# erthward/geonomics

Measured on AMD Instinct MI355X. Metric: individual-timesteps/sec, higher is better.
Workload: dtype u64

## Files before the change

### geonomics_amd/csrc/gnx_api.hip

```cpp
#include <cmath>
#include <cstdarg>
#include <algorithm>
#include <atomic>
#include <chrono>
#include "gnx_internal.h"
#include "gnx_rng.h"
#include "gnx_compact.h"

static thread_local char g_err[1024] = "";

void gnx_set_error(const char* fmt, ...) {
  va_list ap;
  va_start(ap, fmt);
  vsnprintf(g_err, sizeof(g_err), fmt, ap);
  va_end(ap);
}

extern "C" const char* gnx_last_error(void) { return g_err; }

extern "C" int gnx_words_per_hom(int32_t L) {
  int w = (L + 63) / 64;
  return ((w + 15) / 16) * 16;
}

// ... 980 lines not shown
  for (int t = 0; t < h->cfg.n_traits; ++t)
    if (h->traits[t].n_loci == 0) {
      gnx_set_error("trait %d not set (gnx_set_trait)", t);
      return 1;
    }
  return 0;
}

extern "C" int gnx_pop_dynamics_mate(gnx_state* h, int32_t burn) {
  GNXCHK(need_params(h));
  GNXCHK(check_recomb_ready(h, burn != 0));
  int64_t P = 0, B = 0;
  h->tile2_mode = false;
  GNXCHK(gnx_l_sort_by_cell(h, true));
  int rc_pairs = gnx_l_find_pairs(h, nullptr, &P, true);
  GNXCHK(gnx_wait_permute_rest(h));
  GNXCHK(rc_pairs);
  if (P > 0 && !h->spl_P.valid)
    GNXCHK(gnx_l_density(h, P, h->mid_x, h->mid_y, &h->spl_P, nullptr));
  GNXCHK(gnx_l_mate(h, burn != 0, false, 0, &B));
  h->last_births = B;
  return 0;
}

extern "C" int gnx_pop_dynamics_die(gnx_state* h, int32_t burn, int32_t with_selection) {
  GNXCHK(need_params(h));
  int64_t D = 0;
  GNXCHK(gnx_l_density_N(h));
  GNXCHK(gnx_l_death_probs(h, with_selection != 0 && !burn));
  GNXCHK(gnx_l_mortality(h, nullptr, &D));
  h->last_deaths = D;
  return 0;
}

extern "C" int gnx_pop_dynamics(gnx_state* h, int32_t burn, int32_t with_selection) {
  GNXCHK(gnx_pop_dynamics_mate(h, burn));
  return gnx_pop_dynamics_die(h, burn, with_selection);
}

struct GnxStepTimer {
  std::chrono::steady_clock::time_point t0 = std::chrono::steady_clock::now();
  bool count;
  explicit GnxStepTimer(bool c) : count(c) {}
  ~GnxStepTimer() {
    if (gnx_host_times()) {
      g_host_step_s += std::chrono::duration<double>(std::chrono::steady_clock::now() - t0).count();
      if (count) ++g_host_steps;
    }
  }
};

extern "C" int gnx_step_begin(gnx_state* h, int32_t burn) {
  GNXCHK(need_params(h));
  GNXCHK(check_recomb_ready(h, burn != 0));
  GnxStepTimer timer(true);
  if (h->mort_wait || h->pairs_wait) {
    gnx_set_error("gnx_step_begin: the previous step of this handle was not finished (gnx_step_end)");
    return 1;
  }
  h->tot[0] += 1;
  h->tot[1] += h->N - h->n_ghost;
  h->last_xo_births = 0;
  h->step_burn = burn != 0;
  h->tile2_mode = false;
  if (h->moved_ahead) {
    GNXCHK(gnx_move_ahead_join(h));
  } else if (h->sp.move) {
    h->move_writes_keys = h->sp.mating_radius >= 0;
    int rc = gnx_l_move(h, true, nullptr, nullptr, nullptr, nullptr, true);
    h->move_writes_keys = false;
    GNXCHK(rc);
  } else {
    GNXCHK(gnx_l_age(h));
  }
  GNXCHK(gnx_l_sort_by_cell(h, true));
  int rc_pairs = gnx_l_find_pairs_enqueue(h, nullptr, true);
  GNXCHK(gnx_wait_permute_rest(h));
  return rc_pairs;
}

extern "C" int gnx_step_mid(gnx_state* h, int32_t burn, int32_t with_selection) {
  GnxStepTimer timer(false);
  int64_t P = 0, B = 0;
  GNXCHK(gnx_l_find_pairs_finish(h, &P));
  if (P > 0 && !h->spl_P.valid)
    GNXCHK(gnx_l_density(h, P, h->mid_x, h->mid_y, &h->spl_P, nullptr));
  GNXCHK(gnx_l_mate(h, burn != 0, false, 0, &B));
  h->last_births = B;
  GNXCHK(gnx_l_density_N(h));
  GNXCHK(gnx_l_death_probs(h, with_selection != 0 && !burn));
  return gnx_l_mortality_enqueue(h, nullptr);
}

extern "C" int gnx_step_end(gnx_state* h, int32_t burn) {
  GnxStepTimer timer(false);
  int64_t D = 0;
  GNXCHK(gnx_l_mortality_finish(h, &D));
  h->last_deaths = D;
  h->step += 1;
  h->tot[2] += h->last_births;
  h->tot[3] += h->last_deaths;
  if (!burn) h->tot[4] += h->last_xo_births;
  return 0;
}

extern "C" int gnx_step(gnx_state* h, int32_t burn, int32_t with_selection) {
  GNXCHK(gnx_step_begin(h, burn));
  GNXCHK(gnx_step_mid(h, burn, with_selection));
  return gnx_step_end(h, burn);
}

extern "C" int gnx_step_many(gnx_state** hs, int32_t n, int32_t burn, int32_t with_selection) {
  for (int k = 0; k < n; ++k) GNXCHK(gnx_step_begin(hs[k], burn));
  for (int k = 0; k < n; ++k) GNXCHK(gnx_step_mid(hs[k], burn, with_selection));
  for (int k = 0; k < n; ++k) GNXCHK(gnx_step_end(hs[k], burn));
  return 0;
}

extern "C" int gnx_set_id_order(gnx_state* h, int32_t mode) {
  if (mode != 0 && mode != 1) {
    gnx_set_error("gnx_set_id_order: 0 (hash cell, focal id) or 1 (virtual-tile-major)");
    return 1;
  }
  if (mode == 1 && (h->cfg.W % 8 || h->cfg.H % 8)) {
    gnx_set_error("tile-major offspring ids need landscape dimensions divisible by 8");
    return 1;
  }
  if (mode == 1) GNXCHK(gnx_vt_buffers(h));
  h->id_order = mode;
  h->cfg_epoch += 1;
  return 0;
}

extern "C" int gnx_totals(gnx_state* h, int64_t* out) {
  for (int k = 0; k < 6; ++k) out[k] = h->tot[k];
  return 0;
}

extern "C" int gnx_reset_totals(gnx_state* h) {
  for (int k = 0; k < 6; ++k) h->tot[k] = 0;
  return 0;
}

extern "C" int gnx_path_counts(gnx_state* h, int64_t* out, int32_t n) {
  for (int k = 0; k < n; ++k) out[k] = k < GNX_PC_COUNT ? h->pc[k] : 0;
  return GNX_PC_COUNT;
}

extern "C" int gnx_reset_path_counts(gnx_state* h) {
  for (int k = 0; k < GNX_PC_COUNT; ++k) h->pc[k] = 0;
  return 0;
}

__global__ void k_gather_births(int64_t B, int64_t first, GnxSoA s, const int32_t* off_parent,
                                int64_t* child_id, int64_t* parent_id, float* xy) {
  int64_t k = (int64_t)blockIdx.x * blockDim.x + threadIdx.x;
  if (k >= B) return;
  child_id[k] = s.id[first + k];
  parent_id[2 * k] = s.id[off_parent[2 * k]];
  parent_id[2 * k + 1] = s.id[off_parent[2 * k + 1]];
  xy[2 * k] = s.x[first + k];
  xy[2 * k + 1] = s.y[first + k];
}

extern "C" int gnx_last_births(gnx_state* h, int64_t* child_id, int64_t* parent_id, int32_t* keys,
                               uint8_t* starts, float* xy) {
  const int64_t B = h->last_births;
  if (B <= 0) return 0;
  if (B > h->N) {
    gnx_set_error("gnx_last_births: call it between gnx_pop_dynamics_mate and _die");
// ... 457 lines not shown
```

### geonomics_amd/csrc/gnx_internal.h

```cpp
#pragma once
#include <cstring>
#include <cstdint>
#include <cstdio>
#include <cstdlib>
#include <string>
#include <vector>
#include <utility>
#include <hip/hip_runtime.h>
#include "../../include/gnx_hip.h"
#include "gnx_half.h"

#define GNX_MAX_TRAITS 16
#define GNX_MAX_LAYERS 16
#define GNX_DISP_ATTEMPTS 8
#define GNX_SPARSE_MAX_BP 24

void gnx_set_error(const char* fmt, ...);

static inline int gnx_env_int(const char* name, int dflt) {
  const char* v = getenv(name);
  return v ? atoi(v) : dflt;
}
static inline int64_t gnx_dd_max_cap() {
  static const int64_t v = getenv("GNX_DD_MAX_CAP") ? atoll(getenv("GNX_DD_MAX_CAP")) : 600000;
// ... 382 lines not shown
  int32_t* req_count = nullptr;
  bool tiled = false;
  int tile_R = 1, tile_C = 1, tile_r = 0, tile_c = 0;
  gnx_ind_rec* st_rec = nullptr;
  float* st_z = nullptr;
  uint64_t* st_geno = nullptr;
  int64_t* st_slots = nullptr;
  int64_t st_n = 0, st_cap = 0, st_geno_cap = 0;
  bool st_has_geno = false;
  int64_t birth_first_slot = 0;
  int64_t n_req = 0;
  gnx_ind_rec* gp_rec = nullptr;
  float* gp_z = nullptr;
  int64_t* gp_slots = nullptr;
  int64_t gp_cap = 0;
  void* rq_sorted = nullptr;
  int32_t* rq_k = nullptr;
  int64_t rq_cap = 0;
  uint64_t* gam_out = nullptr;
  int32_t* gam_slot = nullptr;
  int64_t gam_cap = 0;
  int64_t* chk = nullptr;
  int64_t tile_evict = 0;
  float evict_box[4]{};
  int64_t n_req_known = -1;
  gnx_ind_rec* gh_rec = nullptr;
  int64_t gh_cap = 0;
  int32_t* route_cnt = nullptr;
  int64_t route_n_mig = 0, route_n_gh = 0;
  int64_t prev_deaths = 0;
  int32_t* h_route_pin = nullptr;
  int32_t* h_route_pin_dev = nullptr;
  std::vector<int64_t> req_by_rank;
  bool tile_req_on_device = false;
  bool tile2_mode = false;
  bool req_cnt_zeroed = false;
  bool tile_pairs_nowait = false;
  bool tile_births_settled = false;

  int32_t* mate = nullptr;
  int32_t* flag = nullptr;
  int32_t* flag2 = nullptr;
  int32_t* scan = nullptr;
  int32_t* pairs = nullptr;
  int32_t* nbirths = nullptr;
  int32_t* boff = nullptr;
  int32_t* off_pair = nullptr;
  int32_t* off_parent = nullptr;
  int32_t* off_keys = nullptr;
  uint8_t* off_start = nullptr;
  uint8_t* keep_in = nullptr;
  float* inj_a = nullptr;
  float* inj_b = nullptr;
  float* mid_x = nullptr;
  float* mid_y = nullptr;
  int64_t n_pairs = 0;
  bool pairs_wait = false;
  int64_t pairs_seq = 0;
  bool pairs_with_top = false, pairs_with_density = false;
  bool mort_wait = false;
  bool mort_xo = false, mort_fill = false, mort_ord_keep = false;
  int mort_has_rows = 0;
  int64_t mort_N = 0;

  GnxLattice lat;
  GnxSpline spl_N, spl_P;
  int32_t* bin_partials = nullptr;
  int32_t* bins_P = nullptr;
  bool bins_zeroed[2]{};
  bool nmax_zeroed = false;
  bool req_zeroed = false;
  int32_t* fb[3]{};
  bool fb_zero[3]{};
  int fb_cur = 0;
  bool fb_adults = false;
  int64_t fb_count = 0;
  unsigned long long* nmax2 = nullptr;
  const unsigned long long* nmax_cur = nullptr;
  bool nmax_ready = false;
  bool last_N_fused = false;
  hipEvent_t ev_pairs = nullptr, ev_latP = nullptr, ev_perm = nullptr, ev_binsN = nullptr;
  bool binsN_inflight = false;
  bool latP_inflight = false;
  bool ord_mode = true;
  bool ord_valid = false;
  int64_t ord_n = 0;
  int ord_cur = 0;
  int32_t* ord[2]{};
  int32_t* newslot = nullptr;
  bool compact_fill = true;
  bool jobs_self_scan = false;
  bool ord_covers_xo = false;
  bool permute_split = true;
  bool perm_rest_inflight = false;
  bool perm_rest_pending = false;
  GnxSoA perm_rest_a{}, perm_rest_b{};
  int64_t perm_rest_N = 0;
  hipEvent_t ev_perm_rest = nullptr;
  bool fb_pending = false;
  const float *fbp_x = nullptr, *fbp_y = nullptr;
  int64_t fbp_N = 0;
  hipEvent_t ev_alive = nullptr;
  int32_t* fill_cnt = nullptr;
  hipEvent_t ev_fill = nullptr;
  int64_t fill_guess = 0;
  uint32_t* cell32 = nullptr;
  uint32_t* keyk[2]{};
  int32_t* valk[2]{};
  void* os_scratch = nullptr;
  uint32_t* os_ktmp = nullptr;
  int32_t* os_vtmp = nullptr;
  int32_t* ord_cnt = nullptr;
  int32_t* ord_off = nullptr;
  hipEvent_t ev_ord = nullptr;
  bool ord_inflight = false;
  bool keys_ordmode = false;
  bool keys_fresh = false;
  bool hist_fresh = false;
  bool holes = false;
  int64_t holes_N = 0;
  RouteGeo* route_geo_dev = nullptr;
  uint64_t route_geo_epoch = 0;
  bool move_counts_routes = false;
  bool move_counted_routes = false;
  bool tile_lazy_ok = false;
  int64_t holes_flagged = 0;
  bool eager_move = false;
  bool move_ahead_ok = false;
  bool moved_ahead = false;
  hipEvent_t ev_moved = nullptr;
  bool e_stale = false;
  bool move_writes_keys = false;
  int n_bin_blocks = 0;
  double* nodes = nullptr;
  double* K_over = nullptr;
  unsigned long long* nmax_bits = nullptr;
  double* p_death = nullptr;
  double* d_cell = nullptr;
  uint8_t* dead_in = nullptr;
  int32_t* counts_rast[2]{};
  int counts_cur = 0;
  bool counts_init = false;
  double* red = nullptr;

  int32_t* blk_cnt = nullptr;
  int32_t* blk_off = nullptr;
  int blk_stride = 0;
  int32_t* cnt_dev = nullptr;
  unsigned int* tickets = nullptr;

  int64_t* h_pin = nullptr;
  int64_t* h_pin_dev = nullptr;
  int64_t pin_seq = 0;
  void* h_stage = nullptr;
  size_t h_stage_bytes = 0;

  void* tile_comm = nullptr;
  GnxDD* dd = nullptr;
  GnxDDRec* dd_ring = nullptr;
  GnxDDRec* dd_ring_dev = nullptr;
  bool dd_active = false;
  int64_t dd_seq = 0;
  int64_t dd_seen = 0;
  int64_t dd_half_est = 0;
  int64_t dd_b_hi = 0;
  int64_t dd_use_hi = 0;
  int64_t dd_gc_seq = 0;
  int64_t dd_top_last = 0, dd_top_seq = 0;
  int64_t dd_est_seq = 0;
  int64_t dd_post_gc = 0;
  bool dd_gc_wait = false;
  void* dd_graph[1]{};
  int32_t dd_err = 0;
  std::vector<int64_t> dd_hist;
  bool dd_hist_closed = false;
  uint64_t cfg_epoch = 1;

  bool profiling = false;
  int profile_only = -1;
  GnxKernelTimer timers[GNX_K_COUNT];
  hipEvent_t ev_open = nullptr;
  std::vector<hipEvent_t> ev_free;
  std::vector<std::pair<hipEvent_t, hipEvent_t>> ev_pending[GNX_K_COUNT];
};

GnxTraitTab gnx_trait_tab(const gnx_state* h);

static inline GnxHalves gnx_halves(const gnx_state* h) {
  return GnxHalves{h->hmap, h->half_free, h->half_top, h->NB, h->BW > 0 ? h->BW : h->W64 / h->NB};
}
int gnx_half_reserve(gnx_state* h, int64_t blocks);
int gnx_gc(gnx_state* h);
static inline const int32_t* gnx_alias_bp(const gnx_state* h) {
  return (h->alias_xo && h->sparse_paths) ? h->bp_off : nullptr;
}
static inline const int32_t* gnx_alias_loci(const gnx_state* h) {
  return (h->alias_xo && h->sparse_paths) ? h->bp_loci : nullptr;
}

int gnx_publish(gnx_state* h, int slot, const int32_t* a, const int32_t* b = nullptr,
                const int32_t* c = nullptr, const int32_t* d = nullptr);

void gnx_time_begin(gnx_state* h, int kernel = -1);
void gnx_time_end(gnx_state* h, int kernel, double bytes);

int gnx_h2d(gnx_state* h, void* dst, const void* src, size_t bytes);
int gnx_d2h(gnx_state* h, void* dst, const void* src, size_t bytes);

int gnx_l_init_population(gnx_state* h, int64_t N);
int gnx_l_gather_e(gnx_state* h, int64_t first, int64_t n);
int gnx_l_age(gnx_state* h);
int gnx_l_move(gnx_state* h, bool inc_age, const float* inj_theta, const float* inj_dist,
               float* out_theta, float* out_dist, bool apply);
int gnx_l_move_ahead(gnx_state* h, int64_t N);
int gnx_move_ahead_join(gnx_state* h);
int gnx_l_sort_by_cell(gnx_state* h, bool split_rest = false);
int gnx_wait_permute_rest(gnx_state* h);
int gnx_permute_rest_launch(gnx_state* h);
int gnx_l_find_pairs(gnx_state* h, const uint8_t* d_keep, int64_t* n_pairs_out,
                     bool with_density = false);
int gnx_l_find_pairs_enqueue(gnx_state* h, const uint8_t* d_keep, bool with_density);
int gnx_l_find_pairs_finish(gnx_state* h, int64_t* n_pairs_out);
int gnx_l_births(gnx_state* h, int64_t* births_out);
int gnx_l_pair_cls(gnx_state* h, int64_t P, bool local);
int gnx_vt_buffers(gnx_state* h);
int gnx_l_mate(gnx_state* h, bool burn, bool inject, int64_t B_inject, int64_t* births_out,
               int64_t id_base = -1, bool tiled = false);
int gnx_l_dispersal_inject(gnx_state* h, int64_t B, int A, const float* d_mx, const float* d_my,
                           const float* d_theta, const float* d_dist, float* d_ox, float* d_oy,
                           int32_t* d_used);
int gnx_l_crossover_all(gnx_state* h, int64_t first_slot, int64_t B);
int gnx_l_crossover_requests(gnx_state* h, int64_t first_slot, int64_t n_req);
int gnx_l_crossover_pending(gnx_state* h, int64_t first_slot, int64_t B);
int gnx_l_crossover_survivors(gnx_state* h, int64_t first_slot, int64_t B, const int32_t* d_alive,
                              const int32_t* d_scan);
int gnx_xo_join(gnx_state* h);
int gnx_xo_flush_deferred(gnx_state* h);
int gnx_xo_launch_pending(gnx_state* h, int site = GNX_PC_XO_FLUSH);
int gnx_xo_wait_inflight(gnx_state* h);
int gnx_xo_prepare_jobs(gnx_state* h, int32_t** zero);
int gnx_xo_wait_wide(gnx_state* h);
double gnx_xo_bytes_per_birth(const gnx_state* h);
int gnx_l_rebuild_sel(gnx_state* h);
int gnx_l_path_sel(gnx_state* h);
int gnx_l_tb_from_rows(gnx_state* h, int64_t first, int64_t n, const int32_t* d_list,
                       const int64_t* d_slots, bool join = true);
int gnx_l_newborn_tb(gnx_state* h, int64_t first_slot, int64_t B);
int gnx_l_phenotype(gnx_state* h, int64_t first_slot, int64_t n, const int32_t* d_list = nullptr);
int gnx_l_assign_genomes(gnx_state* h, const int32_t* d_n_per_site);
int gnx_l_mutate(gnx_state* h, int n, const int64_t* d_slot, const int32_t* d_locus,
                 const uint8_t* d_hom);
int gnx_l_density(gnx_state* h, int64_t n, const float* d_x, const float* d_y, GnxSpline* spl,
                  const double* d_nodes_override, const int32_t* n_dev = nullptr);
struct GnxSetWords {
  int32_t* dst = nullptr;
  int32_t v[4] = {0, 0, 0, 0};
};
struct GnxPubWords {
  int n1 = 0;
  const int32_t* src1 = nullptr;
  int32_t* host1 = nullptr;
  int n2 = 0;
  const int32_t* src2 = nullptr;
  int32_t* host2 = nullptr;
};
int gnx_l_bins(gnx_state* h, int64_t n, const float* d_x, const float* d_y, const uint8_t* d_ghost,
               int32_t* d_bins, const int32_t* n_dev = nullptr, const GnxSetWords* sw = nullptr);
int gnx_l_spline(gnx_state* h, const int32_t* d_bins, GnxSpline* spl,
                 const double* d_nodes_override);
int gnx_l_spline_z(gnx_state* h, const int32_t* d_bins, GnxSpline* spl,
                   const double* d_nodes_override, bool housekeeping);
int gnx_l_raster(gnx_state* h, int which, double* d_out);
int gnx_l_density_N(gnx_state* h);
int gnx_l_lattice_P_async(gnx_state* h, int64_t n_max);
int gnx_bins_adults_launch(gnx_state* h);
void gnx_bins_adults_drop(gnx_state* h);
int gnx_l_bins_adults_async(gnx_state* h, const float* d_x, const float* d_y, int64_t N);
int gnx_wait_latP(gnx_state* h);
bool gnx_fused_bins(const gnx_state* h);
int gnx_l_death_probs(gnx_state* h, bool with_selection);
int gnx_l_mortality(gnx_state* h, const uint8_t* d_dead_inject, int64_t* deaths_out);
int gnx_l_mortality_enqueue(gnx_state* h, const uint8_t* d_dead_inject);
int gnx_l_mortality_finish(gnx_state* h, int64_t* deaths_out);
int gnx_l_spatial_diff(gnx_state* h, double* mean, double* sd, double* sums = nullptr);
int gnx_l_gather_genomes(gnx_state* h, int64_t n, const int64_t* d_slots, uint64_t* d_out);
int gnx_l_scatter_genomes(gnx_state* h, int64_t n, const uint64_t* d_in, int64_t first_slot);

int gnx_dd_l_sort(gnx_state* h, int32_t* d_bins, hipStream_t st);
int gnx_dd_l_pairs(gnx_state* h, int32_t* d_bins, hipStream_t st);
int gnx_dd_l_offspring(gnx_state* h, bool genomes, int32_t* d_bins, hipStream_t st);
int gnx_dd_l_density_N(gnx_state* h, int par, hipStream_t st);
int gnx_dd_l_death_probs(gnx_state* h, bool with_selection, int par, hipStream_t st);
int gnx_dd_l_alive(gnx_state* h, bool xo, int buf, hipStream_t st);
int gnx_dd_l_jobs(gnx_state* h, int buf, hipStream_t st);
int gnx_dd_l_crossover(gnx_state* h, int buf, hipStream_t st);
int gnx_dd_l_fill_lists(gnx_state* h, int has_rows, hipStream_t st);
int gnx_dd_l_fill(gnx_state* h, int has_rows, bool xo, hipStream_t st);
int gnx_dd_l_ord_end(gnx_state* h, int has_rows, bool xo, hipStream_t st);
bool gnx_dd_eligible(const gnx_state* h, bool burn);
int gnx_dd_leave(gnx_state* h);
void gnx_dd_destroy(gnx_state* h);

int gnx_block_scan(gnx_state* h, int K, int64_t n_items, const int32_t* cnt, int32_t* off,
                   int32_t* out, int64_t* host, int64_t seq = 0, hipStream_t st = nullptr,
                   const int32_t* extra = nullptr);
int gnx_os_hist_discard(gnx_state* h, hipStream_t st = nullptr);
bool gnx_l_lattices_tiled(gnx_state* h, bool have_pairs, const GnxPubWords& pub);
void gnx_host_mark(int id);
extern double g_host_step_s, g_host_wait_s;
bool gnx_host_times();
size_t gnx_os_scratch_bytes(size_t n, int end_bit);
size_t gnx_os_words_used64(size_t n, int end_bit);
int gnx_os_sort64_clean(void* scratch, void* tmp, const uint64_t* kin, uint64_t* kout,
                        const int32_t* vin, int32_t* vout, size_t n, int end_bit, hipStream_t s);
size_t gnx_os_words_used(size_t n, int end_bit);
int gnx_os_keys_hist(void* scratch, unsigned int* ticket, int64_t N, int64_t ord_n,
                     const int32_t* ord, const uint32_t* cell32, uint32_t* key, int32_t* val,
                     int end_bit, hipStream_t s, const GnxDD* dd = nullptr, int geometry = 0);
void gnx_os_digits(int end_bit, int* places, int* rb);
int gnx_os_sort32_gather(void* scratch, uint32_t* ktmp, int32_t* vtmp, uint32_t* kout, int32_t* vout,
                         size_t n, int end_bit, const int32_t* ord, int64_t ord_n,
// ... 93 lines not shown
```

### geonomics_amd/csrc/gnx_kernels_genome.hip

```cpp
#include "gnx_internal.h"
#include "gnx_rng.h"
#include "gnx_xo.h"
#include "gnx_half.h"
#include "gnx_tb.h"
#include "gnx_compact.h"

__global__ void __launch_bounds__(256)
k_xo_jobs_all(int64_t B, int64_t first, int32_t* __restrict__ grow,
              const int32_t* __restrict__ off_parent, const int32_t* __restrict__ off_keys,
              const uint8_t* __restrict__ off_start, const int32_t* __restrict__ free_rows,
              int64_t n_free, GnxHalves H, const int32_t* __restrict__ bp_off,
              const int32_t* __restrict__ bp_loci, GnxXoJob* __restrict__ jobs,
              int32_t* __restrict__ n_jobs) {
  const int64_t k = (int64_t)blockIdx.x * blockDim.x + threadIdx.x;
  const bool act = k < B;
  int32_t row = -1;
  if (act) {
    row = free_rows[n_free - 1 - k];
    grow[first + k] = row;
  }
#pragma unroll
  for (int p = 0; p < 2; ++p) {
    const int32_t prow = act ? grow[off_parent[2 * k + p]] : -1;
    gnx_xo_gamete(H, act, row, p, prow, act ? off_keys[2 * k + p] : 0,
// ... 166 lines not shown
        jrec.ph0 = GNX_BLK(pe0[b]);
        jrec.ph1 = GNX_BLK(pe1[b]);
        jrec.dst = dst;
        jrec.ks = (key * 2 + st) | (b << 24);
        jobs[job++] = jrec;
      }
    } else {
      const int hsel = (sel >> b) & 1u;
      const int32_t e = hsel ? pe1[b] : pe0[b];
      H.hmap[lb] = GNX_BLK(e);
      if (e < 0) H.hmap[((int64_t)prow * 2 + hsel) * NB + b] = GNX_BLK(e);
    }
  }
  for (int b = 0; b < NB; ++b)
    H.hmap[((int64_t)row * 2 + 1) * NB + b] = (int32_t)((uint32_t)H.stack[pop - nf0 - b] | GNX_OWN);
}

int gnx_l_crossover_requests(gnx_state* h, int64_t first_slot, int64_t n_req) {
  if (n_req == 0) return 0;
  GNXCHK(gnx_xo_launch_pending(h));
  GNXCHK(xo_wait_buf(h, h->stream, 0));
  GNXCHK(xo_wait_buf(h, h->stream, 1));
  const int buf = h->jobs_cur;
  GNXCHK(gnx_half_reserve(h, 2 * (int64_t)h->NB * n_req));
  HIPCHK(hipMemsetAsync(h->n_jobs_dev[buf], 0, sizeof(int32_t), h->stream));
  h->jobs_inline[buf] = false;
  hipLaunchKernelGGL(k_xo_jobs_req, dim3(gnx_grid(n_req, 256)), dim3(256), 0, h->stream, (int)n_req,
                     first_slot, h->soa[h->cur].grow, h->req_k, h->off_parent, h->off_keys,
                     h->off_start, h->free_rows, h->n_free, gnx_halves(h), gnx_alias_bp(h),
                     gnx_alias_loci(h), (GnxXoJob*)h->jobs[buf], h->n_jobs_dev[buf]);
  if (h->stream2) {
    HIPCHK(hipEventRecord(h->ev_jobs, h->stream));
    HIPCHK(hipStreamWaitEvent(h->stream2, h->ev_jobs, 0));
  }
  gnx_time_begin(h, GNX_K_CROSSOVER);
  GNXCHK(xo_launch(h, h->stream, buf, n_req, false));
  gnx_time_end(h, GNX_K_CROSSOVER, 0.0);
  h->n_free -= n_req;
  return 0;
}

__global__ void k_pending_flags(int64_t N, int64_t first, const int32_t* grow, int32_t* alive,
                                int32_t* cnt3) {
  __shared__ int lds[16];
  const int64_t base = (int64_t)blockIdx.x * GNX_CB;
  bool fx[4];
#pragma unroll
  for (int r = 0; r < 4; ++r) {
    const int64_t i = base + r * 256 + threadIdx.x;
    fx[r] = i < N && i >= first && grow[i] < 0;
    if (i < N) alive[i] = fx[r] ? 2 : 0;
  }
  int rank[4], tot;
  gnx_block_ranks(fx, rank, tot, lds);
  if (threadIdx.x == 0) cnt3[blockIdx.x] = tot;
}

int gnx_l_crossover_pending(gnx_state* h, int64_t first_slot, int64_t B) {
  if (B == 0) return 0;
  GNXCHK(gnx_xo_launch_pending(h));
  GNXCHK(xo_wait_buf(h, h->stream, 0));
  GNXCHK(xo_wait_buf(h, h->stream, 1));
  const int64_t N = h->N;
  const int nb = (int)((N + GNX_CB - 1) / GNX_CB);
  const int buf = h->jobs_cur;
  int32_t* cnt3 = h->blk_cnt + 2 * h->blk_stride;
  int32_t* off3 = h->blk_off + 2 * h->blk_stride;
  hipLaunchKernelGGL(k_pending_flags, dim3(nb), dim3(256), 0, h->stream, N, first_slot,
                     h->soa[h->cur].grow, h->flag, cnt3);
  GNXCHK(gnx_block_scan(h, 1, N, cnt3, off3, h->cnt_dev + 2, h->h_pin_dev + 8));
  GNXCHK(gnx_half_reserve(h, 2 * (int64_t)h->NB * B));
  HIPCHK(hipMemsetAsync(h->n_jobs_dev[buf], 0, sizeof(int32_t), h->stream));
  gnx_launch_xo_jobs_surv(h, first_slot, h->flag, h->blk_off, buf);
  gnx_time_begin(h, GNX_K_CROSSOVER);
  GNXCHK(xo_launch(h, h->stream, buf, 2 * B, false));
  HIPCHK(hipStreamSynchronize(h->stream));
  const int64_t S = h->h_pin[8];
  gnx_time_end(h, GNX_K_CROSSOVER, 0.0);
  h->n_free -= S;
  h->last_xo_births = S;
  return 0;
}

int gnx_xo_launch_pending(gnx_state* h, int site) {
  const int buf = h->xo_ready_buf;
  if (buf < 0) return 0;
  h->xo_ready_buf = -1;
  if (site == GNX_PC_XO_P2 || site == GNX_PC_XO_FLUSH) ++h->pc[site];
  HIPCHK(hipEventRecord(h->ev_jobs, h->stream));
  HIPCHK(hipStreamWaitEvent(h->stream2, h->ev_jobs, 0));
  hipStream_t main = h->stream;
  h->stream = h->stream2;
  const int split = (h->xo_sort_waits && h->xo_split > 0 && h->xo_split < 1024) ? h->xo_split : 0;
  h->xo_last_split = split;
  gnx_time_begin(h, GNX_K_CROSSOVER);
  int rc = xo_launch(h, h->stream2, buf, h->xo_ready_jobs, !h->xo_sort_waits, 0,
                     split ? split : 1024);
  gnx_time_end(h, GNX_K_CROSSOVER, 0.0);
  if (split && !rc) {
    HIPCHK(hipEventRecord(h->ev_xo_wide[buf], h->stream2));
    h->xo_wide_inflight[buf] = true;
    gnx_time_begin(h, GNX_K_CROSSOVER);
    rc = xo_launch(h, h->stream2, buf, h->xo_ready_jobs, true, split, 1024);
    gnx_time_end(h, GNX_K_CROSSOVER_TAIL, 0.0);
  }
  h->stream = main;
  GNXCHK(rc);
  HIPCHK(hipEventRecord(h->ev_xo_done[buf], h->stream2));
  h->xo_inflight[buf] = true;
  h->xo_running = true;
  return 0;
}

int gnx_xo_wait_inflight(gnx_state* h) {
  GNXCHK(xo_wait_buf(h, h->stream, 0));
  GNXCHK(xo_wait_buf(h, h->stream, 1));
  return 0;
}

int gnx_xo_wait_wide(gnx_state* h) {
  for (int buf = 0; buf < 2; ++buf) {
    if (h->xo_wide_inflight[buf]) {
      HIPCHK(hipStreamWaitEvent(h->stream, h->ev_xo_wide[buf], 0));
      h->xo_wide_inflight[buf] = false;
    } else if (!h->xo_last_split) {
      GNXCHK(xo_wait_buf(h, h->stream, buf));
    }
  }
  return 0;
}

int gnx_xo_prepare_jobs(gnx_state* h, int32_t** zero) {
  GNXCHK(gnx_xo_launch_pending(h));
  const int buf = h->jobs_cur;
  GNXCHK(xo_wait_buf(h, h->stream, buf));
  *zero = h->n_jobs_dev[buf];
  return 0;
}

int gnx_l_crossover_survivors(gnx_state* h, int64_t first_slot, int64_t B, const int32_t* d_alive,
                              const int32_t* d_scan) {
  if (B == 0) return 0;
  const int buf = h->jobs_cur;
  gnx_launch_xo_jobs_surv(h, first_slot, d_alive, d_scan, buf);
  HIPCHK(hipGetLastError());
  h->xo_ready_buf = buf;
  h->xo_ready_jobs = 2 * B;
  h->jobs_cur ^= 1;
  if (!h->xo_launch_late || h->tiled || h->tile2_mode) GNXCHK(gnx_xo_launch_pending(h, -1));
  return 0;
}

int gnx_xo_flush_deferred(gnx_state* h) {
  if (h->xo_deferred) {
    GNXCHK(gnx_xo_launch_pending(h));
    h->xo_deferred = false;
    GNXCHK(gnx_l_crossover_pending(h, h->xo_first, h->xo_B));
  }
  return 0;
}

int gnx_xo_join(gnx_state* h) {
  GNXCHK(gnx_xo_flush_deferred(h));
  GNXCHK(gnx_xo_launch_pending(h));
  GNXCHK(xo_wait_buf(h, h->stream, 0));
  GNXCHK(xo_wait_buf(h, h->stream, 1));
  return 0;
}

__global__ void k_path_sel(int n_paths, int TW, int n_sel, int W64, const int32_t* sel_loci,
                           const u64* paths, u64* out) {
  const int idx = blockIdx.x * blockDim.x + threadIdx.x;
  if (idx >= n_paths * TW) return;
// ... 462 lines not shown
```

### geonomics_amd/csrc/gnx_kernels_pop.hip

```cpp
#include "gnx_internal.h"
#include "gnx_rng.h"
#include "gnx_compact.h"
#include "gnx_tb.h"
#include "gnx_bins.h"

static int gnx_id_bits(const gnx_state* h) {
  int b = 1;
  while (b < 40 && (h->max_id >> b) != 0) ++b;
  return b;
}
static bool gnx_ord_sort(const gnx_state* h) {
  return h->ord_mode && h->ord_valid && !h->tiled;
}

__device__ __forceinline__ int wave_min_i(int v) {
#pragma unroll
  for (int m = 32; m >= 1; m >>= 1) v = min(v, __shfl_xor(v, m));
  return v;
}
__device__ __forceinline__ int wave_max_i(int v) {
#pragma unroll
  for (int m = 32; m >= 1; m >>= 1) v = max(v, __shfl_xor(v, m));
  return v;
}
// ... 1580 lines not shown
  if (threadIdx.x < GNX_VTN) {
    const int t = vtot[threadIdx.x];
    vt.blk_cnt[(int64_t)threadIdx.x * vt.stride + blockIdx.x] = t;
    if (t) atomicAdd(&vt.total[threadIdx.x], t);
    const unsigned long long nz = __ballot(t != 0);
    if (threadIdx.x == 0) vt.blk_nz[blockIdx.x] = nz;
  }
}

__global__ void __launch_bounds__(256)
k_pair_compact(int64_t N, const int32_t* focal, const int32_t* mate, const int32_t* flag2,
               const int32_t* blk_off, const float* x, const float* y, const uint64_t* popkey,
               int idbits, int32_t* pairs, float* mid_x, float* mid_y, uint64_t* key,
               const int32_t* __restrict__ cnt, int32_t* __restrict__ total_dev,
               int64_t* __restrict__ host, long long seq, const int32_t* __restrict__ extra,
               GnxDD* __restrict__ dd, int dd_births, int64_t dd_cap, GnxBinP bins, GnxVtOut vt) {
  __shared__ int lds[16];
  __shared__ int psum[4];
  __shared__ int vcnt[16][GNX_VTN];
  __shared__ int vpre[GNX_VTN];
  if (dd) N = dd->N;
  if (vt.cls) {
    for (int k = threadIdx.x; k < 16 * GNX_VTN; k += 256) (&vcnt[0][0])[k] = 0;
    const int lane = threadIdx.x & 63, wave = threadIdx.x >> 6;
    unsigned long long nz = vt.blk_nz[blockIdx.x];
    for (int k = 0; nz; ++k) {
      const int c = __ffsll((long long)nz) - 1;
      nz &= nz - 1;
      if ((k & 3) != wave) continue;
      const int32_t* row = vt.blk_cnt + (int64_t)c * vt.stride;
      int part = 0;
      for (int b2 = lane; b2 < (int)blockIdx.x; b2 += 64) part += row[b2];
#pragma unroll
      for (int d = 32; d > 0; d >>= 1) part += __shfl_xor(part, d);
      if (lane == 0) vpre[c] = part;
    }
    if (vt.local && blockIdx.x == 0 && wave == 3) {
      const int tot = vt.total[lane];
      int xs = tot;
#pragma unroll
      for (int d = 1; d < 64; d <<= 1) {
        const int yv = __shfl_up(xs, d);
        if (lane >= d) xs += yv;
      }
      vt.base[lane] = (int64_t)(xs - tot) * vt.lam;
    }
  }
  int self_off = 0;
  if (cnt) {
    const int lane = threadIdx.x & 63, wave = threadIdx.x >> 6;
    const int upto = blockIdx.x == 0 ? (int)gridDim.x : (int)blockIdx.x;
    int part = 0;
    for (int i = threadIdx.x; i < upto; i += 256) part += cnt[i];
#pragma unroll
    for (int d = 32; d > 0; d >>= 1) part += __shfl_xor(part, d);
    if (lane == 0) psum[wave] = part;
    __syncthreads();
    const int sum = psum[0] + psum[1] + psum[2] + psum[3];
    self_off = blockIdx.x == 0 ? 0 : sum;
    if (blockIdx.x == 0 && threadIdx.x == 0) {
      *total_dev = sum;
      if (dd) {
        int64_t births = (int64_t)sum * dd_births;
        if ((int64_t)dd->N + births > dd_cap) {
          dd->err |= GNX_DD_ERR_SLOTS;
          births = 0;
        }
        dd->P = sum;
        dd->B = (int32_t)births;
      }
      if (host) {
        __hip_atomic_store(&host[0], (int64_t)sum, __ATOMIC_RELAXED, __HIP_MEMORY_SCOPE_SYSTEM);
        if (extra)
          __hip_atomic_store(&host[12], (int64_t)*extra, __ATOMIC_RELAXED, __HIP_MEMORY_SCOPE_SYSTEM);
        asm volatile("s_waitcnt vmcnt(0)" ::: "memory");
        if (seq)
          __hip_atomic_store(&host[3], (int64_t)seq, __ATOMIC_RELAXED, __HIP_MEMORY_SCOPE_SYSTEM);
      }
    }
  }
  const int64_t base = (int64_t)blockIdx.x * GNX_CB;
  bool f[4];
  int sc[4] = {0, 0, 0, 0};
#pragma unroll
  for (int r = 0; r < 4; ++r) {
    const int64_t i = base + r * 256 + threadIdx.x;
    f[r] = i < N && flag2[i] != 0;
    if (vt.cls && i < N) sc[r] = vt.scls[i];
  }
  int rank[4], tot;
  gnx_block_ranks(f, rank, tot, lds);
  int vc[4] = {0, 0, 0, 0}, vrw[4] = {0, 0, 0, 0};
  float fx[4], fy[4];
  int fo4[4];
#pragma unroll
  for (int r = 0; r < 4; ++r) {
    const int64_t i = base + r * 256 + threadIdx.x;
    fo4[r] = f[r] ? (focal ? focal[i] : (int)i) : 0;
    fx[r] = f[r] ? x[fo4[r]] : 0.f;
    fy[r] = f[r] ? y[fo4[r]] : 0.f;
  }
  if (vt.cls) {
    const int lane = threadIdx.x & 63, wave = threadIdx.x >> 6;
#pragma unroll
    for (int r = 0; r < 4; ++r) {
      vc[r] = f[r] ? sc[r] : GNX_VTN;
      gnx_vt_wave_ranks<false>(f[r], vc[r], 1, lane, vcnt[r * 4 + wave], vrw[r]);
    }
    __syncthreads();
  }
  const int32_t bo = cnt ? self_off : blk_off[blockIdx.x];
#pragma unroll
  for (int r = 0; r < 4; ++r) {
    const int64_t i = base + r * 256 + threadIdx.x;
    int bin = 0;
    if (f[r]) {
      const int p = bo + rank[r];
      const int m = mate[i];
      const int fo = fo4[r];
      pairs[2 * p] = fo;
      pairs[2 * p + 1] = m;
      const float mx = (fx[r] + x[m]) / 2.0f, my = (fy[r] + y[m]) / 2.0f;
      mid_x[p] = mx;
      mid_y[p] = my;
      const uint64_t k = popkey[i];
      key[p] = ((k >> idbits) << 40) | (k & ((1ull << idbits) - 1ull));
      if (bins.bins) bin = gnx_bin_of(bins, mx, my);
      if (vt.cls) {
        const int wave = threadIdx.x >> 6;
        int before = vpre[vc[r]];
        for (int j = 0; j < r * 4 + wave; ++j) before += vcnt[j][vc[r]];
        vt.cls[p] = (uint8_t)vc[r];
        vt.rank[p] = before + vrw[r];
      }
    }
    if (bins.bins) gnx_bin_add(bins.bins, bin, f[r]);
  }
}

__global__ void k_panmixia(int64_t N, const int64_t* id, long long step, unsigned long long seed,
                           int32_t* focal, int32_t* mate) {
  int64_t i = (int64_t)blockIdx.x * blockDim.x + threadIdx.x;
  if (i >= N) return;
  uint4 r = gnx_rand4(seed, (unsigned long long)id[i], step, OP_PAIR_KEEP, 1);
  int f = (int)(((unsigned long long)r.x * (unsigned long long)N) >> 32);
  int m = (int)(((unsigned long long)r.y * (unsigned long long)N) >> 32);
  focal[i] = f;
  mate[i] = (m == f) ? -1 : m;
}

int gnx_l_find_pairs(gnx_state* h, const uint8_t* d_keep, int64_t* n_pairs_out, bool with_density) {
  int rc = gnx_l_find_pairs_enqueue(h, d_keep, with_density);
  if (rc) {
    *n_pairs_out = 0;
    return rc;
  }
  return gnx_l_find_pairs_finish(h, n_pairs_out);
}

constexpr int GNX_FM_EASY_ROUNDS = 2;

int gnx_l_find_pairs_enqueue(gnx_state* h, const uint8_t* d_keep, bool with_density) {
  int64_t N = h->N;
  h->n_pairs = 0;
  h->pairs_wait = false;
  if (N == 0) return 0;
  const gnx_species_params& sp = h->sp;
  GnxSoA s = h->soa[h->cur];
  int sexed = sp.sexed;
  const int32_t* focal = nullptr;
  gnx_time_begin(h);
  if (sp.mating_radius < 0) {
    focal = h->off_pair;
    hipLaunchKernelGGL(k_panmixia, dim3(gnx_grid(N, 256)), dim3(256), 0, h->stream, N, s.id,
                       h->step, h->cfg.seed, h->off_pair, h->mate);
  } else {
    float r = (float)sp.mating_radius;
    float r2 = r * r;
    FocalP fp{N, d_keep, (float)sp.b, sexed, sp.repro_age[0], h->step, h->cfg.seed};
    dim3 grid(gnx_grid(N, FM_PER_BLOCK)), blk(256);
    const uint4* cd = (const uint4*)h->cand;
    if (sp.mate_mode == GNX_MATE_NEAREST)
      hipLaunchKernelGGL(k_find_mates<GNX_MATE_NEAREST>, grid, blk, 0, h->stream, fp, s, cd,
                         h->inv_cs, h->cell_start, h->ncx, h->ncy, h->cell_ref, r, r2, GNX_FM_EASY_ROUNDS, h->mate);
    else if (sp.mate_mode == GNX_MATE_INVERSE)
      hipLaunchKernelGGL(k_find_mates<GNX_MATE_INVERSE>, grid, blk, 0, h->stream, fp, s, cd,
                         h->inv_cs, h->cell_start, h->ncx, h->ncy, h->cell_ref, r, r2, GNX_FM_EASY_ROUNDS, h->mate);
    else
      hipLaunchKernelGGL(k_find_mates<GNX_MATE_UNIFORM>, grid, blk, 0, h->stream, fp, s, cd,
                         h->inv_cs, h->cell_start, h->ncx, h->ncy, h->cell_ref, r, r2, GNX_FM_EASY_ROUNDS, h->mate);
  }
  gnx_time_end(h, GNX_K_FIND_MATES, (double)N * 16.0);
  GNXCHK(gnx_permute_rest_launch(h));
  gnx_time_begin(h);
  const int nb = (int)((N + GNX_CB - 1) / GNX_CB);
  PairP pp{N, focal, h->mate, d_keep, (float)sp.b, sexed, sp.repro_age[0], sp.repro_age[1],
           (sexed || sp.mating_radius < 0) ? 0 : 1,
           h->step, h->cfg.seed};
  GnxVtOut vto;
  GNXCHK(gnx_vt_out(h, &vto));
  hipLaunchKernelGGL(k_pair_flags, dim3(nb), dim3(256), 0, h->stream, pp, s, h->flag2, h->blk_cnt, vto);
  const int64_t seq = ++h->pin_seq;
  const bool with_top = h->half_top && h->genomes_assigned;
  hipLaunchKernelGGL(k_pair_compact, dim3(nb), dim3(256), 0, h->stream, N, focal, h->mate,
                     h->flag2, h->blk_off, s.x, s.y, h->key64[1], gnx_id_bits(h), h->pairs,
                     h->mid_x, h->mid_y, h->key64[0],
                     (const int32_t*)h->blk_cnt, h->cnt_dev,
                     h->h_pin_dev + 4, (long long)seq,
                     with_top ? (const int32_t*)h->half_top : (const int32_t*)nullptr,
                     (GnxDD*)nullptr, 0, (int64_t)0, GnxBinP{nullptr, 0.0, 0, 0}, vto);
  gnx_time_end(h, GNX_K_PAIRS, (double)N * 40.0);
  HIPCHK(hipGetLastError());
  if (with_density && gnx_fused_bins(h)) {
    GNXCHK(gnx_l_lattice_P_async(h, N));
  } else if (with_density) {
    const bool lds_bins = (size_t)h->lat.nbx * h->lat.nby * sizeof(int32_t) <= 48 * 1024;
    if (lds_bins)
      GNXCHK(gnx_l_density(h, N, h->mid_x, h->mid_y, &h->spl_P, nullptr, h->cnt_dev));
    else
      with_density = false;
  }
  h->pairs_wait = true;
  h->pairs_seq = seq;
  h->pairs_with_top = with_top;
  h->pairs_with_density = with_density;
  return 0;
}

int gnx_l_find_pairs_finish(gnx_state* h, int64_t* n_pairs_out) {
  *n_pairs_out = 0;
  if (!h->pairs_wait) return 0;
  h->pairs_wait = false;
  GNXCHK(gnx_wait_published(h, 4, h->pairs_seq));
  h->n_pairs = h->h_pin[4];
  if (h->pairs_with_top) h->half_free_est = h->h_pin[16];
  *n_pairs_out = h->n_pairs;
  if (!h->pairs_with_density) h->spl_P.valid = false;
  else if (h->n_pairs == 0) h->spl_P.valid = false;
  if (h->xo_launch_late) GNXCHK(gnx_xo_launch_pending(h, GNX_PC_XO_P2));
  return 0;
}

__global__ void k_births(int64_t P, const int32_t* pairs, const int64_t* id, float thr,
                         long long step, unsigned long long seed, int32_t* nb) {
  int64_t p = (int64_t)blockIdx.x * blockDim.x + threadIdx.x;
  if (p >= P) return;
  GnxStream st(seed, (unsigned long long)id[pairs[2 * p]], step, OP_BIRTHS);
  int k = 0;
  float prod = 1.0f;
  for (int j = 0; j < 64; ++j) {
    prod = prod * gnx_u01(st.next());
    if (!(prod > thr)) break;
    k++;
  }
  nb[p] = max(k, 1);
}

__global__ void k_expand_births(int64_t P, const int32_t* nb, const int32_t* boff,
                                int32_t* off_pair) {
  int64_t p = (int64_t)blockIdx.x * blockDim.x + threadIdx.x;
  if (p >= P) return;
  int o = boff[p];
  for (int q = 0; q < nb[p]; ++q) off_pair[o + q] = (int32_t)p;
}

struct OffP {
  int64_t N, B, cap;
  int W, H, n_layers;
  float xmax, ymax, rrx, rry;
  int distr;
  float p1, p2;
  int surf, surf_layer;
  float surf_kappa;
  int sexed;
  float p_male;
  int fixed_nb;
  int genomes;
  int n_paths;
  int64_t id_base, n_free;
  long long step;
  unsigned long long seed;
  int fuse_tb, TW;
  const uint64_t* path_sel;
  const uint8_t* dom;
  GnxBinP bins;
  const GnxDD* dd;
  const uint64_t* ptb;
  const int32_t* pmap;
  const int32_t* P_dev;
};

struct GnxReq {
  int64_t* pid;
  int32_t* k;
  int32_t* key;
  uint8_t* start;
  float* px;
  float* py;
  int32_t* count;
};

__device__ __forceinline__ bool disperse_once(float mx, float my, float theta, float dist,
                                              float rrx, float rry, float xmax, float ymax,
                                              float& ox, float& oy) {
  float dx = cosf(theta) * dist;
  float dy = sinf(theta) * dist;
  if (rrx != 1.0f) dx *= rrx;
  if (rry != 1.0f) dy *= rry;
  ox = fminf(fmaxf(mx + dx, 0.0f), xmax);
  oy = fminf(fmaxf(my + dy, 0.0f), ymax);
  return ox > 0.0f && oy > 0.0f;
}

__global__ void __launch_bounds__(256)
k_offspring(OffP P, GnxSoA s, const float* rast, const int32_t* pairs, const int32_t* off_pair,
            const int32_t* boff, GnxGoff gf,
            int32_t* off_parent, int32_t* off_keys, uint8_t* off_start, GnxReq rq, GnxTraitTab T,
            int32_t* __restrict__ ord_tail) {
  int64_t k = (int64_t)blockIdx.x * blockDim.x + threadIdx.x;
  if (P.dd) {
    P.N = P.dd->N;
    P.B = P.dd->B;
// ... 431 lines not shown
```

Measured before the change: 2.588 billion.

## Launch pending crossover after births on pairs event; prefetch pair compaction loads

In the mid step, the pending crossover launch on the secondary stream is now deferred until after mating is enqueued, and it waits on an event recorded right after pair compaction instead of the current stream tail. The aim is to let births/mating kernels get ahead on the main stream while crossover overlaps. Separately, k_pair_compact now loads flag, mate, focal, key and coordinates for all four rows up front with clamped indices, so loads issue before the block rank scan rather than being gated by flags. This adds extra loads for unflagged lanes and more register pressure, plus new conditions governing when the event is recorded.

```diff
diff --git a/geonomics_amd/csrc/gnx_api.hip b/geonomics_amd/csrc/gnx_api.hip
--- a/geonomics_amd/csrc/gnx_api.hip
+++ b/geonomics_amd/csrc/gnx_api.hip
@@ -1086,10 +1086,20 @@
 extern "C" int gnx_step_mid(gnx_state* h, int32_t burn, int32_t with_selection) {
   GnxStepTimer timer(false);
   int64_t P = 0, B = 0;
-  GNXCHK(gnx_l_find_pairs_finish(h, &P));
+  const bool counted = h->pairs_wait;
+  GNXCHK(gnx_l_find_pairs_count(h, &P));
+  const bool held = counted && h->xo_launch_late && h->xo_ready_buf >= 0;
+  const bool births_first =
+      held && h->pairs_ev && !h->xo_deferred && !h->tiled && h->sp.n_births_fixed;
+  if (held && !births_first) GNXCHK(gnx_xo_launch_pending(h, GNX_PC_XO_P2));
   if (P > 0 && !h->spl_P.valid)
     GNXCHK(gnx_l_density(h, P, h->mid_x, h->mid_y, &h->spl_P, nullptr));
-  GNXCHK(gnx_l_mate(h, burn != 0, false, 0, &B));
+  int rc = gnx_l_mate(h, burn != 0, false, 0, &B);
+  if (births_first) {
+    const int rc_xo = gnx_xo_launch_pending(h, GNX_PC_XO_P2, h->ev_pairs);
+    if (!rc) rc = rc_xo;
+  }
+  GNXCHK(rc);
   h->last_births = B;
   GNXCHK(gnx_l_density_N(h));
   GNXCHK(gnx_l_death_probs(h, with_selection != 0 && !burn));
diff --git a/geonomics_amd/csrc/gnx_internal.h b/geonomics_amd/csrc/gnx_internal.h
--- a/geonomics_amd/csrc/gnx_internal.h
+++ b/geonomics_amd/csrc/gnx_internal.h
@@ -488,6 +488,7 @@
   hipEvent_t ev_pairs = nullptr, ev_latP = nullptr, ev_perm = nullptr, ev_binsN = nullptr;
   bool binsN_inflight = false;
   bool latP_inflight = false;
+  bool pairs_ev = false;
   bool ord_mode = true;
   bool ord_valid = false;
   int64_t ord_n = 0;
@@ -627,6 +628,7 @@
                      bool with_density = false);
 int gnx_l_find_pairs_enqueue(gnx_state* h, const uint8_t* d_keep, bool with_density);
 int gnx_l_find_pairs_finish(gnx_state* h, int64_t* n_pairs_out);
+int gnx_l_find_pairs_count(gnx_state* h, int64_t* n_pairs_out);
 int gnx_l_births(gnx_state* h, int64_t* births_out);
 int gnx_l_pair_cls(gnx_state* h, int64_t P, bool local);
 int gnx_vt_buffers(gnx_state* h);
@@ -642,7 +644,7 @@
                               const int32_t* d_scan);
 int gnx_xo_join(gnx_state* h);
 int gnx_xo_flush_deferred(gnx_state* h);
-int gnx_xo_launch_pending(gnx_state* h, int site = GNX_PC_XO_FLUSH);
+int gnx_xo_launch_pending(gnx_state* h, int site = GNX_PC_XO_FLUSH, hipEvent_t after = nullptr);
 int gnx_xo_wait_inflight(gnx_state* h);
 int gnx_xo_prepare_jobs(gnx_state* h, int32_t** zero);
 int gnx_xo_wait_wide(gnx_state* h);
diff --git a/geonomics_amd/csrc/gnx_kernels_genome.hip b/geonomics_amd/csrc/gnx_kernels_genome.hip
--- a/geonomics_amd/csrc/gnx_kernels_genome.hip
+++ b/geonomics_amd/csrc/gnx_kernels_genome.hip
@@ -272,13 +272,16 @@
   return 0;
 }
 
-int gnx_xo_launch_pending(gnx_state* h, int site) {
+int gnx_xo_launch_pending(gnx_state* h, int site, hipEvent_t after) {
   const int buf = h->xo_ready_buf;
   if (buf < 0) return 0;
   h->xo_ready_buf = -1;
   if (site == GNX_PC_XO_P2 || site == GNX_PC_XO_FLUSH) ++h->pc[site];
-  HIPCHK(hipEventRecord(h->ev_jobs, h->stream));
-  HIPCHK(hipStreamWaitEvent(h->stream2, h->ev_jobs, 0));
+  if (!after) {
+    HIPCHK(hipEventRecord(h->ev_jobs, h->stream));
+    after = h->ev_jobs;
+  }
+  HIPCHK(hipStreamWaitEvent(h->stream2, after, 0));
   hipStream_t main = h->stream;
   h->stream = h->stream2;
   const int split = (h->xo_sort_waits && h->xo_split > 0 && h->xo_split < 1024) ? h->xo_split : 0;
diff --git a/geonomics_amd/csrc/gnx_kernels_pop.hip b/geonomics_amd/csrc/gnx_kernels_pop.hip
--- a/geonomics_amd/csrc/gnx_kernels_pop.hip
+++ b/geonomics_amd/csrc/gnx_kernels_pop.hip
@@ -1686,24 +1686,34 @@
   const int64_t base = (int64_t)blockIdx.x * GNX_CB;
   bool f[4];
   int sc[4] = {0, 0, 0, 0};
-#pragma unroll
-  for (int r = 0; r < 4; ++r) {
-    const int64_t i = base + r * 256 + threadIdx.x;
-    f[r] = i < N && flag2[i] != 0;
-    if (vt.cls && i < N) sc[r] = vt.scls[i];
-  }
+  int32_t fl[4] = {0, 0, 0, 0}, mt[4] = {0, 0, 0, 0}, fo4[4] = {0, 0, 0, 0};
+  uint64_t pk[4] = {0, 0, 0, 0};
+  float fx[4] = {0.f, 0.f, 0.f, 0.f}, fy[4] = {0.f, 0.f, 0.f, 0.f};
+  float gx[4] = {0.f, 0.f, 0.f, 0.f}, gy[4] = {0.f, 0.f, 0.f, 0.f};
+  if (base < N) {
+#pragma unroll
+    for (int r = 0; r < 4; ++r) {
+      const int64_t ic = min(base + r * 256 + (int64_t)threadIdx.x, N - 1);
+      fl[r] = flag2[ic];
+      mt[r] = mate[ic];
+      fo4[r] = focal ? focal[ic] : (int32_t)ic;
+      pk[r] = popkey[ic];
+      if (vt.cls) sc[r] = vt.scls[ic];
+    }
+#pragma unroll
+    for (int r = 0; r < 4; ++r) {
+      const int32_t mc = mt[r] >= 0 ? mt[r] : fo4[r];
+      fx[r] = x[fo4[r]];
+      fy[r] = y[fo4[r]];
+      gx[r] = x[mc];
+      gy[r] = y[mc];
+    }
+  }
+#pragma unroll
+  for (int r = 0; r < 4; ++r) f[r] = base + r * 256 + threadIdx.x < N && fl[r] != 0;
   int rank[4], tot;
   gnx_block_ranks(f, rank, tot, lds);
   int vc[4] = {0, 0, 0, 0}, vrw[4] = {0, 0, 0, 0};
-  float fx[4], fy[4];
-  int fo4[4];
-#pragma unroll
-  for (int r = 0; r < 4; ++r) {
-    const int64_t i = base + r * 256 + threadIdx.x;
-    fo4[r] = f[r] ? (focal ? focal[i] : (int)i) : 0;
-    fx[r] = f[r] ? x[fo4[r]] : 0.f;
-    fy[r] = f[r] ? y[fo4[r]] : 0.f;
-  }
   if (vt.cls) {
     const int lane = threadIdx.x & 63, wave = threadIdx.x >> 6;
 #pragma unroll
@@ -1716,18 +1726,15 @@
   const int32_t bo = cnt ? self_off : blk_off[blockIdx.x];
 #pragma unroll
   for (int r = 0; r < 4; ++r) {
-    const int64_t i = base + r * 256 + threadIdx.x;
     int bin = 0;
     if (f[r]) {
       const int p = bo + rank[r];
-      const int m = mate[i];
-      const int fo = fo4[r];
-      pairs[2 * p] = fo;
-      pairs[2 * p + 1] = m;
-      const float mx = (fx[r] + x[m]) / 2.0f, my = (fy[r] + y[m]) / 2.0f;
+      pairs[2 * p] = fo4[r];
+      pairs[2 * p + 1] = mt[r];
+      const float mx = (fx[r] + gx[r]) / 2.0f, my = (fy[r] + gy[r]) / 2.0f;
       mid_x[p] = mx;
       mid_y[p] = my;
-      const uint64_t k = popkey[i];
+      const uint64_t k = pk[r];
       key[p] = ((k >> idbits) << 40) | (k & ((1ull << idbits) - 1ull));
       if (bins.bins) bin = gnx_bin_of(bins, mx, my);
       if (vt.cls) {
@@ -1768,6 +1775,7 @@
   int64_t N = h->N;
   h->n_pairs = 0;
   h->pairs_wait = false;
+  h->pairs_ev = false;
   if (N == 0) return 0;
   const gnx_species_params& sp = h->sp;
   GnxSoA s = h->soa[h->cur];
@@ -1815,7 +1823,13 @@
                      (GnxDD*)nullptr, 0, (int64_t)0, GnxBinP{nullptr, 0.0, 0, 0}, vto);
   gnx_time_end(h, GNX_K_PAIRS, (double)N * 40.0);
   HIPCHK(hipGetLastError());
-  if (with_density && gnx_fused_bins(h)) {
+  const bool fused = with_density && gnx_fused_bins(h);
+  h->pairs_ev = fused;
+  if (!fused && h->xo_launch_late && h->xo_ready_buf >= 0 && !h->tiled && !h->tile2_mode) {
+    HIPCHK(hipEventRecord(h->ev_pairs, h->stream));
+    h->pairs_ev = true;
+  }
+  if (fused) {
     GNXCHK(gnx_l_lattice_P_async(h, N));
   } else if (with_density) {
     const bool lds_bins = (size_t)h->lat.nbx * h->lat.nby * sizeof(int32_t) <= 48 * 1024;
@@ -1832,6 +1846,13 @@
 }
 
 int gnx_l_find_pairs_finish(gnx_state* h, int64_t* n_pairs_out) {
+  const bool waited = h->pairs_wait;
+  GNXCHK(gnx_l_find_pairs_count(h, n_pairs_out));
+  if (waited && h->xo_launch_late) GNXCHK(gnx_xo_launch_pending(h, GNX_PC_XO_P2));
+  return 0;
+}
+
+int gnx_l_find_pairs_count(gnx_state* h, int64_t* n_pairs_out) {
   *n_pairs_out = 0;
   if (!h->pairs_wait) return 0;
   h->pairs_wait = false;
@@ -1841,7 +1862,6 @@
   *n_pairs_out = h->n_pairs;
   if (!h->pairs_with_density) h->spl_P.valid = false;
   else if (h->n_pairs == 0) h->spl_P.valid = false;
-  if (h->xo_launch_late) GNXCHK(gnx_xo_launch_pending(h, GNX_PC_XO_P2));
   return 0;
 }
 
```

Result: faster. 2.640 billion, median of 6 (+2.0%).
